# lmfaber/karma

Measured on AMD Instinct MI355X. Metric: contigs+reads/sec for k-mer vec + shared-read graph build; HBM GB/s vs roofline, higher is better.
Workload: dtype u32 keys / i64 counts / f64 div

## Files before the change

### include/karma.h

```cpp
#ifndef KARMA_H
#define KARMA_H

#include <stddef.h>
#include <stdint.h>

#ifdef __cplusplus
extern "C" {
#endif

#define KARMA_OK 0
#define KARMA_ERR_ARG (-1)
#define KARMA_ERR_KMER (-2)
#define KARMA_ERR_HIP (-3)
#define KARMA_ERR_OOM (-4)
#define KARMA_ERR_ZERO_DIV (-5)
#define KARMA_ERR_UNSORTED (-6)
#define KARMA_ERR_STATE (-7)
#define KARMA_ERR_PARSE (-8)
#define KARMA_ERR_COMM (-9)
#define KARMA_ERR_STALL (-10)

#define KARMA_KMER_5P6 (-1)

int karma_version(void);
// ... 79 lines not shown
int karma_ctx_join(karma_ctx* ctx, void* side);
int karma_ctx_set_side_headroom(karma_ctx* ctx, int blocks_per_cu);
int karma_kmer_row_totals(karma_kmer_plan* p, int64_t* dst_host);

typedef struct karma_pairs karma_pairs;
#define KARMA_REC_SORTED 0
#define KARMA_REC_UNSORTED 1
#define KARMA_REC_FLAGGED 2
int karma_graph_records(karma_ctx* ctx, const uint32_t* records, int64_t n_records, int64_t n_contigs, int flags,
                        int is_device, karma_pairs** out);
typedef struct karma_graph_job karma_graph_job;
int karma_graph_records_begin(karma_ctx* ctx, const uint32_t* records, int64_t n_records, int64_t n_contigs,
                              int flags, int is_device, karma_graph_job** job);
int karma_graph_records_end(karma_graph_job* job, karma_pairs** out);
int karma_graph_split_hint(karma_ctx* ctx, const int64_t* bounds, int nranks);
int karma_graph_eq(karma_ctx* ctx, const int64_t* cls_off, const uint32_t* members, const int64_t* counts,
                   const uint8_t* pair_skip, int64_t n_classes, int64_t n_contigs, int is_device, karma_pairs** out);
int karma_graph_eq_compact(karma_ctx* ctx, const uint8_t* sizes, const uint32_t* members, int64_t n_members,
                           const uint32_t* counts, int64_t C, int64_t n_contigs, karma_pairs** out);
int karma_pairs_merge(karma_ctx* ctx, const uint64_t* keys, const int64_t* counts, int64_t n, int is_device,
                      karma_pairs** out);
int karma_pairs_merge_runs(karma_ctx* ctx, const uint64_t* keys, const int64_t* counts, const int64_t* run_off,
                           int n_runs, int is_device, karma_pairs** out);
int karma_pairs_get_kc(karma_pairs* p, int64_t* kc_dev);
int karma_pairs_merge_runs_kc(karma_ctx* ctx, const int64_t* kc_dev, const int64_t* run_off, int n_runs,
                              karma_pairs** out);
int karma_pairs_destroy(karma_pairs* p);
int karma_pairs_rebind(karma_pairs* p, karma_ctx* ctx);
int karma_pairs_count(karma_pairs* p, int64_t* n);
int karma_pairs_device(karma_pairs* p, const uint64_t** keys, const int64_t** counts);
// ... 105 lines not shown
```

### karma_amd/_lib.py

```python

from __future__ import annotations

import ctypes
import os
import weakref

import numpy as np

HERE = os.path.dirname(os.path.abspath(__file__))
LIB_PATH = os.environ.get("KARMA_LIB") or os.path.join(HERE, "libkarma_hip.so")

KARMA_OK = 0
KARMA_ERR_ARG = -1
KARMA_ERR_KMER = -2
KARMA_ERR_HIP = -3
KARMA_ERR_OOM = -4
KARMA_ERR_ZERO_DIV = -5
KARMA_ERR_UNSORTED = -6
KARMA_ERR_STATE = -7
KARMA_ERR_PARSE = -8
KARMA_ERR_COMM = -9
KARMA_ERR_STALL = -10

KARMA_DT_U8, KARMA_DT_I32, KARMA_DT_I64, KARMA_DT_U64, KARMA_DT_F64 = 0, 1, 2, 3, 4
# ... 67 lines not shown
    "karma_kmer_exceptions_set": [_c_p, _c_p, _i64],
    "karma_kmer_plan_finalize": [_c_p, _I64P],
    "karma_kmer_plan_finalize_async": [_c_p],
    "karma_kmer_plan_finalize_wait": [_c_p, _I64P],
    "karma_kmer_columns": [_c_p, _c_p],
    "karma_kmer_profile": [_c_p, _c_p, _i64, _i32],
    "karma_kmer_profile_rows": [_c_p, _i64, _i64, _c_p, _i64, _i32],
    "karma_kmer_profile_side": [_c_p, _c_p, _i64, _c_p],
    "karma_ctx_join": [_c_p, _c_p],
    "karma_ctx_set_side_headroom": [_c_p, _i32],
    "karma_kmer_row_totals": [_c_p, _c_p],
    "karma_graph_records": [_c_p, _c_p, _i64, _i64, _i32, _i32, _PP],
    "karma_graph_records_begin": [_c_p, _c_p, _i64, _i64, _i32, _i32, _PP],
    "karma_graph_records_end": [_c_p, _PP],
    "karma_graph_split_hint": [_c_p, _c_p, _i32],
    "karma_graph_eq": [_c_p, _c_p, _c_p, _c_p, _c_p, _i64, _i64, _i32, _PP],
    "karma_graph_eq_compact": [_c_p, _c_p, _c_p, _i64, _c_p, _i64, _i64, _PP],
    "karma_pairs_merge": [_c_p, _c_p, _c_p, _i64, _i32, _PP],
    "karma_pairs_merge_runs": [_c_p, _c_p, _c_p, _c_p, _i32, _i32, _PP],
    "karma_pairs_merge_runs_kc": [_c_p, _c_p, _c_p, _i32, _PP],
    "karma_pairs_get_kc": [_c_p, _c_p],
    "karma_pairs_destroy": [_c_p],
    "karma_pairs_rebind": [_c_p, _c_p],
    "karma_pairs_count": [_c_p, _I64P],
    "karma_pairs_device": [_c_p, _PP, _PP],
    "karma_pairs_get": [_c_p, _c_p, _c_p, _c_p, _i32],
    "karma_pairs_split": [_c_p, _c_p, _i32, _c_p],
    "karma_pairs_totals": [_c_p, _c_p, _i64],
    "karma_edges_from_pairs": [_c_p, _c_p, _i32, _c_p, _i64, _PP, _I64P],
    "karma_edges_begin": [_c_p, _c_p, _i32, _i64, _PP, _PP],
# ... 309 lines not shown
```

### karma_amd/csrc/graph_sets.hip

```cpp

#include <algorithm>
#include <cstdlib>
#include <cstring>
#include <memory>
#include <type_traits>

#include "karma_internal.h"
#include "sets_ctrl.h"

using namespace karma;

namespace {

#include "graph_device.h"

typedef unsigned int u32x4 __attribute__((ext_vector_type(4)));

constexpr int kMaxB = 2048;
constexpr int kMaxBc = 512;
constexpr int kNarrowB = 512, kNarrowBc = 128;
constexpr int kCrSmax = 64;
constexpr int kCrPieces = 512;
constexpr int kCgShift = 18;
constexpr int kOneGroupB = 128;
// ... 134 lines not shown
                                               uint32_t* m0_out) {
    const uint32_t za = (uint32_t)__builtin_ctz(a.win), zb = (uint32_t)__builtin_ctz(b.win);
    const uint32_t ma = a.fm3 + za, mb = b.fm3 + zb, m0 = min(ma, mb);
    const uint32_t rel = ((a.win >> za) << min(ma - m0, 31u)) | ((b.win >> zb) << min(mb - m0, 31u));
    *code = K23 ? m0 << 4 | rel : m0 | (rel >> 1) << 24;
    *m0_out = m0;
    return COMPACT ? lanes(rel < 16u) & (K23 ? ~0ull : lanes(m0 < N)) : 0ull;
}

__device__ __forceinline__ uint32_t dpp_shr1(uint32_t old, uint32_t v) {
    return (uint32_t)__builtin_amdgcn_update_dpp((int)old, (int)v, 0x138, 0xF, 0xF, false);
}

constexpr int kRareMax = int(kCChunk / kCIter);
constexpr int kRareW = 5;
#ifndef KARMA_CLS_PACKED
#define KARMA_CLS_PACKED 0
#endif
constexpr int kCls2Waves = 4;

constexpr int kBinQ = 64;
constexpr int kBinMaxBc = 56;
constexpr int kBinHdr = 4;
struct BinArgs {
    uint16_t* segs;
    uint4* hdr;
    uint8_t* dir;
    int64_t seg_cap;
    int dir_cap;
    int slotted;
};

template <bool HIST, bool COMPACT, bool REMAP = false, bool BIN = false, bool FLAG = false>
__global__ void __launch_bounds__(kCW) __attribute__((amdgpu_waves_per_eu(kCls2Waves, kCls2Waves)))
classify2_kernel(ClassArgs P, BinArgs Q) {
    static_assert(!(HIST && BIN), "the binned classify has no partition block histograms");
    auto PA = [&]() -> const ClassArgs& {
        const char* ka = (const char*)__builtin_amdgcn_kernarg_segment_ptr();
        asm volatile("" : "+s"(ka));
        return *reinterpret_cast<const ClassArgs*>(ka);
    };
    constexpr int RPL = FLAG ? 16 : 8;
    constexpr int64_t kIt = 64 * RPL;
    constexpr int kFPer = RPL / 4;
    static_assert(!FLAG || kFPer <= kCPer, "the step's units fit the register set");
    constexpr bool RC = BIN && FLAG;
    constexpr bool RAW = FLAG;
    constexpr bool PK = RC && KARMA_CLS_PACKED;
    constexpr uint32_t kWinTop = PK ? 7u : 31u;
    const int lane = threadIdx.x & 63;
    const int wave = __builtin_amdgcn_readfirstlane(threadIdx.x >> 6);
    const int64_t chunk = P.c0 + (int64_t)blockIdx.x * (kCW / 64) + wave;
    const int64_t c_lo = chunk * P.chunk;
    if (c_lo >= P.A) return;
    const int64_t c_hi = min(P.A, c_lo + P.chunk);
    uint32_t* out = P.codes + c_lo;
    const uint64_t out_u = (uint64_t)out;
    const __amdgpu_buffer_rsrc_t out_rsrc = __builtin_amdgcn_make_buffer_rsrc(
        reinterpret_cast<void*>(((uint64_t)(uint32_t)__builtin_amdgcn_readfirstlane((int)(out_u >> 32)) << 32) |
                                (uint32_t)__builtin_amdgcn_readfirstlane((int)(uint32_t)out_u)),
        0, (int)(P.chunk * 4), 0x00020000);
    constexpr int kRows = BIN ? 32 : 64;
    __shared__ __attribute__((aligned(16))) u32x4 tbuf[kCW / 64][kRows * 4];
    u32x4* tb = tbuf[wave];
    __shared__ uint32_t whist[kCW / 64][HIST ? kMaxBc : 1];
    uint32_t* wh = whist[wave];
    __shared__ __attribute__((aligned(16))) uint16_t bq[kCW / 64][BIN ? kBinMaxBc * kBinQ : 8];
    __shared__ uint32_t bcnt[kCW / 64][BIN ? kBinMaxBc : 1];
    uint16_t* const q = bq[wave];
    uint32_t* const qn = bcnt[wave];
    __shared__ uint32_t bback[kCW / 64][BIN ? 8 : 1];
    uint32_t* const bst = bback[wave];
    __shared__ uint32_t rlist[kCW / 64][kRareMax * kRareW];
    uint32_t* const rl = rlist[wave];
    uint32_t n_rare = 0;
    constexpr bool hist_on = HIST;
    if (hist_on) {
        for (int b = lane; b < P.Bc; b += 64) wh[b] = 0;
        wave_sync();
    }
    if (BIN) {
        if (lane < P.Bc) qn[lane] = 0;
        if (lane < 8) bst[lane] = 0;
        wave_sync();
// ... 27 lines not shown
            }
            if (lane == 0) {
                Qa.dir[chunk * Qa.dir_cap + nbk] = (uint8_t)fb;
                bst[0] = nbk + 1;
                bst[1 + (fb >> 5)] |= 1u << (fb & 31);
                if (nbk < 16) bst[3 + (nbk >> 2)] |= fb << (8 * (nbk & 3));
            }
            wave_lds_order();
            if (in_mask(over) && bk == fb) q[fb * kBinQ + pos - kBinQ] = val;
            if (lane == 0) qn[fb] -= (uint32_t)kBinQ;
            wave_lds_order();
        }
    };
    uint32_t* const stg = reinterpret_cast<uint32_t*>(tb);
    const uint32_t* const stg_l = stg + lane;
    uint32_t ns = 0;
    uint32_t nc = 0, ng = 0;
    auto stage = [&](uint64_t b, uint32_t v) {
        if (in_mask(b)) stg[ns + (uint32_t)rank_below(b)] = v;
        ns += __popcll(b);
    };
    static_assert(kBinQ == 64, "queue slots: bk << 6");
    uint64_t stage_hi = 0, hi_next = 0;
    const uint32_t code_hi = ((uint32_t)max(P.N, 3u) - 3u) << 4;
    auto bin_stage = [&]() {
        if (!ns) return;
        wave_lds_order();
        for (uint32_t j0 = 0; j0 < ns; j0 += 64) {
            uint32_t cd = stg_l[j0];
            uint64_t m = lanes((uint32_t)lane < ns - j0);
// ... 60 lines not shown
#pragma unroll
            for (int u = 0; u < kFPer; ++u) b[u] = u32x4{rm(b[u].x), rm(b[u].y), rm(b[u].z), rm(b[u].w)};
            return;
        }
#pragma unroll
        for (int u = 0; u < kCPer; ++u) {
            b[u].y = b[u].y < P.N ? P.remap[b[u].y] : b[u].y;
            b[u].w = b[u].w < P.N ? P.remap[b[u].w] : b[u].w;
        }
    };
    auto step = [&](auto full_tag, auto replay_tag, u32x4 (&buf)[kCPer], u32x4 (&nxt)[kCPer], int64_t t0) {
        constexpr bool FULL = decltype(full_tag)::value;
        constexpr bool REPLAY = decltype(replay_tag)::value;
        uint32_t rid[RPL], ctg[RPL];
        if constexpr (FLAG) {
            const int rl = lane & 31;
#pragma unroll
            for (int h = 0; h < 2; ++h) {
#pragma unroll
                for (int u = 0; u < 2; ++u) {
                    const int g = 64 * u + lane;
                    tb[g ^ ((g >> 4) & 3)] = buf[2 * h + u];
                }
                wave_sync();
                if ((lane >> 5) == h) {
#pragma unroll
                    for (int k = 0; k < 4; ++k) {
                        const int g = 4 * rl + k;
                        const u32x4 qv = tb[g ^ ((g >> 4) & 3)];
                        rid[4 * k] = qv.x, rid[4 * k + 1] = qv.y, rid[4 * k + 2] = qv.z, rid[4 * k + 3] = qv.w;
                    }
                }
                wave_sync();
            }
#pragma unroll
            for (int i = 0; i < RPL; ++i) ctg[i] = rid[i] & kContigMask;
        } else if (!BIN) {
#pragma unroll
            for (int u = 0; u < kCPer; ++u) {
                const int row = 16 * u + (lane >> 2);
// ... 103 lines not shown
            auto S = [&](int i) -> uint64_t {
                if (FLAG) return lanes((int)rid[i] < 0) | (i == 0 && !have_prev ? 1ull : 0ull);
                return i == 0 ? lanes(rid[0] != prev_last) | (have_prev ? 0ull : 1ull) : lanes(rid[i] != rid[i - 1]);
            };
            const uint64_t S0 = S(0);
            RState hd;
            rs_reset(st, ctg[0]);
            hd = st;
            spos = 0;
            uint32_t hlen = in_mask(S0) ? 0u : (uint32_t)RPL;
            constexpr bool HLEN = RARE || RPL <= 8;
            started = S0;
            uint64_t Si = S0;
#pragma unroll
            for (int i = 0; i < RPL; ++i) {
                if (!RARE && BIN && i == 8) bin_stage();
                if (i > 0) {
                    const uint64_t cap = Si & ~started;
                    hd.win = in_mask(cap) ? st.win : hd.win;
                    if (HLEN) hlen = in_mask(cap) ? (uint32_t)i : hlen;
                    started |= Si;
                    spos = in_mask(Si) ? (uint32_t)i : spos;
                    if (RAW) {
                        const uint32_t w = rid[i];
                        const uint32_t fm3 = in_mask(Si) ? w - 0x80000003u : st.fm3;
                        st.win = in_mask(Si) ? 8u : st.win | (1u << min(w - fm3, kWinTop));
                        st.fm3 = fm3;
                    } else {
                        const uint32_t c = ctg[i];
                        const uint32_t fm3 = in_mask(Si) ? c - 3u : st.fm3;
                        st.win = (in_mask(Si) ? 0u : st.win) | (1u << min(c - fm3, 31u));
// ... 208 lines not shown
        }
        if (lane == 0) {
            uint4* const h = Q.hdr + kBinHdr * chunk;
            h[0] = uint4{0u, 0u, 0u, 0u};
            h[1] = uint4{0u, 0u, 0u, bst[0]};
            h[2] = uint4{bst[1], bst[2], bst[3], bst[4]};
            h[3] = uint4{bst[5], bst[6], nc, 0u};
        }
    } else if (BIN) {
        wave_lds_order();
        const uint32_t cnt = lane < P.Bc ? qn[lane] : 0u;
        const uint32_t g = (cnt + 7u) >> 3;
        const uint32_t incl = wave_scan_incl(g), excl = incl - g;
        const uint32_t G = lane63(incl);
        uint16_t* const gt = reinterpret_cast<uint16_t*>(tb);
        uint8_t* const gb = reinterpret_cast<uint8_t*>(tb) + 1024;
        for (uint32_t i = 0; i < g; ++i) gt[excl + i] = (uint16_t)(lane << 3 | i);
        gb[lane] = (uint8_t)g;
        wave_lds_order();
        for (uint32_t k0 = 0; k0 < G; k0 += 64) {
            const uint32_t k = k0 + lane;
            if (k < G) {
                const uint32_t e = gt[k], bk = e >> 3, i = e & 7u;
                const uint32_t n = qn[bk];
                u32x4 v = *reinterpret_cast<const u32x4*>(q + bk * kBinQ + 8 * i);
                const int k0c = 8 * (int)i;
                auto pad = [&](uint32_t w, int c) -> uint32_t {
                    const uint32_t lo = k0c + c < (int)n ? (w & 0xFFFFu) : 0xFFFFu;
                    const uint32_t hi = k0c + c + 1 < (int)n ? (w >> 16) : 0xFFFFu;
                    return lo | hi << 16;
                };
// ... 1439 lines not shown
int64_t chunk_records(const karma_ctx* ctx, int64_t A) {
    if (const char* e = std::getenv("KARMA_CHUNK")) {
        const int64_t c = std::atoll(e);
        if (c == kCChunk || c == kCChunk / 2 || c == kCChunk / 4) return c;
    }
    const int64_t slots = (int64_t)ctx->cu_count * 16;
    return ceil_div(A, kCChunk) < 4 * slots ? kCChunk / 2 : kCChunk;
}
int mark_at(int asked) {
    static const int env = [] {
        const char* e = std::getenv("KARMA_MARK_AT");
        return e ? std::atoi(e) : -1;
    }();
    return env >= 0 ? env : asked >= 0 ? asked : kMarkAt;
}
template <typename F>
int pick(bool b, F f) {
    return b ? f(std::true_type{}) : f(std::false_type{});
}
struct SetsJob {
    karma_ctx* ctx = nullptr;
    RecIn rec;
    int64_t A = 0, N = 0;
    SetsOpts opts;
    Geo g{};
    int B = 0;
    int64_t n_chunks = 0;
    int64_t chunk = kCChunk;
    bool wide_c = false, wide_p = false, append = false;
    int lpb = 0;
    int64_t n_pblk = 0;
    DevArray<uint32_t> codes, n_codes, n_gen, n_pl;
    DevArray<int64_t> big_list;
// ... 83 lines not shown
    lb = reinterpret_cast<uint64_t*>(cb + cl.lb);
    flags = reinterpret_cast<int*>(cb + cl.flags);
    counters = reinterpret_cast<unsigned*>(cb + cl.counters);
    n_per = cb + cl.n_per;
    dst = cb + cl.dst;
    ovf = reinterpret_cast<uint8_t*>(cb + cl.ovf);
    split_loc = cb + cl.split_loc;
    if (!deferred) {
        void* hpin = nullptr;
        KARMA_TRY(ctx_job_pinned(ctx, cl.readback * 8, &hpin));
        hctrl = static_cast<const int64_t*>(hpin);
    }
    max_cflush = n_pblk + ceil_div(A, CodeStream::kCap) + 1;
    ccap = A + max_cflush * (8 * (int64_t)g.Bc + 8);
    if (append) KARMA_TRY(blk_hist.alloc(ctx, n_pblk * g.Bc));
    bin = !append && g.Bc > 0 && g.Bc <= kBinMaxBc && bin_on();
    if (bin) {
        dir_cap = (int)(chunk / kBinQ);
        seg_cap = (uint32_t)(dir_cap + g.Bc);
        constexpr int kBinSlotMin = 120;
        slotted = A > 0 && chunk >= (int64_t)kBinSlotMin * g.Bc;
        KARMA_CHECK(n_chunks * (int64_t)seg_cap < (int64_t(1) << 32), KARMA_ERR_ARG,
                    "binned classify: %lld chunks exceed 32-bit segment indices", (long long)n_chunks);
        KARMA_TRY(bsegs.alloc(ctx, n_chunks * (int64_t)seg_cap * kBinQ));
        KARMA_TRY(bhdr.alloc(ctx, n_chunks * 4 * kBinHdr));
        KARMA_TRY(bdir.alloc(ctx, n_chunks * (int64_t)dir_cap));
    } else if (g.Bc > 0) {
        KARMA_TRY(cent.alloc(ctx, ccap + 16));
        KARMA_TRY(cf_base.alloc(ctx, max_cflush));
        KARMA_TRY(cf_off.alloc(ctx, max_cflush * (g.Bc + 1)));
    }
// ... 20 lines not shown
    const int64_t pscap = n_chunks * pcap + max_pflush * (4 * (int64_t)B + 4);
    KARMA_TRY(plist.alloc(ctx, n_chunks * pcap));
    KARMA_TRY(pent.alloc(ctx, pscap + 8));
    KARMA_TRY(pf_base.alloc(ctx, max_pflush));
    KARMA_TRY(pf_off.alloc(ctx, max_pflush * (B + 1)));
    const bool fresh_ext = ext && attempt == 0 && !relabeled;
    const bool probe = A > 0 && !relabeled && !fresh_ext;
    if (!probe && !fresh_ext) KARMA_HIP(hipMemsetAsync(cb, 0, cl.total * 8, ctx->stream));
    if (append) KARMA_HIP(hipMemsetAsync(blk_hist.ptr, 0, n_pblk * g.Bc * 4, ctx->stream));
    const int mark_here = mark_at(opts.mark);
    auto mark = [&](int at) -> int {
        if (mark_here != at || attempt != 0) return KARMA_OK;
        if (!ctx->mark_ev) KARMA_HIP(hipEventCreateWithFlags(&ctx->mark_ev, hipEventDisableTiming));
        KARMA_HIP(hipEventRecord(ctx->mark_ev, ctx->stream));
        ctx->mark_set = true;
        return KARMA_OK;
    };
    if (!relabeled) KARMA_TRY(mark(3));
    if (A > 0) {
        ClassArgs C{rec.pr,    A,         (uint32_t)N,   g.Bc > 0,     codes.ptr, n_codes.ptr,
                    n_gen.ptr, blk_items, lpb, big_list.ptr, counters, flags,
                    append ? blk_hist.ptr : nullptr, g.bwc, g.Bc, relabeled ? remap_map.ptr : nullptr, 0, nullptr,
                    chunk};
        C.recw = rec.fw;
        const BinArgs Bn = bin ? BinArgs{bsegs.ptr, reinterpret_cast<uint4*>(bhdr.ptr), bdir.ptr, (int64_t)seg_cap,
                                         dir_cap, slotted ? 1 : 0}
                               : BinArgs{};
        auto classify = [&](int64_t c_from, int64_t c_to) -> int {
            C.c0 = c_from;
            const int64_t cg = ceil_div(c_to - c_from, kCW / 64);
            if (cg <= 0) return KARMA_OK;
            return pick(rec.flagged(), [&](auto fl) -> int {
                auto go = [&](auto ap, auto bn) -> int {
                    return pick(relabeled, [&](auto rl) -> int {
                        KARMA_LAUNCH(ctx, "graph_classify",
                                     (classify2_kernel<decltype(ap)::value, true, decltype(rl)::value,
                                                       decltype(bn)::value, decltype(fl)::value>),
                                     cg, kCW, 0, C, Bn);
                        return KARMA_OK;
                    });
                };
                return bin ? go(std::false_type{}, std::true_type{})
                           : append ? go(std::true_type{}, std::false_type{}) : go(std::false_type{}, std::false_type{});
            });
        };
        if (probe) {
            KARMA_LAUNCH(ctx, "relabel_probe", relabel_probe_kernel, 1, kRelabelProbes, 0, rec, A, (uint32_t)N,
                         counters + kCtrRelabel, reinterpret_cast<uint64_t*>(cb), cl.total);
            C.skip = counters + kCtrRelabel;
        } else if (fresh_ext) {
            C.skip = counters + kCtrRelabel;
            C.vote = counters + kCtrVote;
        }
        KARMA_TRY(classify(0, n_chunks));
    }
    KARMA_TRY(mark(1));
    if (A == 0) {
        KARMA_HIP(hipMemsetAsync(n_codes.ptr, 0, n_chunks * 4, ctx->stream));
// ... 288 lines not shown
void sets_release(SetsJob* job) {
    if (!job) return;
    job->ctx->job_open = false;
    job->ctx->mark_set = false;
    delete job;
}

int records_to_pairs_sets(karma_ctx* ctx, RecIn rec, int64_t A, int64_t N, karma_pairs* out) {
    if (N > kMaxCompactN) return records_to_pairs_wide(ctx, rec, A, N, out);
    SetsJob* job = nullptr;
    KARMA_TRY(sets_begin(ctx, rec, A, N, SetsOpts{}, &job));
    return sets_end(job, out);
}

}
```

### karma_amd/csrc/karma_internal.h

```cpp
#pragma once

#include <hip/hip_runtime.h>

#include <cstdint>
#include <cstdio>
#include <map>
#include <string>
#include <utility>
#include <vector>

#include "../../include/karma.h"

namespace karma {

void set_error(const char* fmt, ...);

extern thread_local uint64_t t_hip_calls;
constexpr bool counted_call(const char* e) {
    return !((e[0] == 'h' && e[1] == 'i' && e[2] == 'p' && e[3] == 'G' && e[4] == 'e' && e[5] == 't' && e[6] == 'L') ||
             (e[0] == 'h' && e[1] == 'i' && e[2] == 'p' && e[3] == 'S' && e[4] == 'e' && e[5] == 't' && e[6] == 'D'));
}

#define KARMA_HIP(expr)                                                                     \
    do {                                                                                    \
// ... 181 lines not shown
namespace karma {
struct RecIn {
    const uint2* pr = nullptr;
    const uint32_t* fw = nullptr;
    __host__ __device__ bool flagged() const { return fw != nullptr; }
    __device__ __forceinline__ uint32_t contig(int64_t i) const { return fw ? fw[i] & 0x7FFFFFFFu : pr[i].y; }
    __device__ __forceinline__ bool cont(int64_t i) const { return fw ? (int)fw[i] >= 0 : pr[i].x == pr[i - 1].x; }
};
int records_to_pairs_sets(karma_ctx* ctx, RecIn rec, int64_t A, int64_t N, karma_pairs* out);
struct SetsOpts {
    hipStream_t fork = nullptr;
    bool single_stream = false;
    int mark = -1;
    int64_t* ctrl = nullptr;
    int64_t ctrl_words = 0;
};
struct SetsJob;
int64_t sets_max_contigs();
int sets_begin(karma_ctx* ctx, RecIn rec, int64_t A, int64_t N, const SetsOpts& opts, SetsJob** job);
int sets_end(SetsJob* job, karma_pairs* out);
void sets_free(SetsJob* job);
struct SetsDeferred {
    const uint64_t* keys = nullptr;
    const int64_t* counts = nullptr;
    int64_t cap = 0;
    const int64_t* dst = nullptr;
    const int64_t* split_loc = nullptr;
    std::vector<int64_t> split_b;
    int B = 0, bw = 0;
    const int* flags = nullptr;
// ... 12 lines not shown
```

### karma_amd/csrc/step.hip

```cpp
#include <algorithm>
#include <chrono>
#include <cstdlib>
#include <cstring>
#include <deque>
#include <initializer_list>
#include <memory>
#include <thread>
#include <vector>

#include "karma_internal.h"
#include "sets_ctrl.h"
#include "step_schedule.h"

using namespace karma;

namespace {

constexpr int kRing = 64;
constexpr int kLag = 3;

enum StepErr : int64_t { kErrOrder = 1, kErrRange = 2, kErrPartition = 4, kErrZeroTotal = 8, kErrMergeOrder = 16 };
struct StepStatus {
    uint64_t seq;
    int64_t slow;
// ... 496 lines not shown
    int64_t* graves_h = nullptr;
    hipEvent_t grave_ev[kRing] = {};
    std::deque<int> graves;
    int grave_next = 0;
    int64_t n_sync = 0, n_deferred = 0, n_redone = 0;
    int64_t run_ns = 0, wait_ns = 0;
    karma_contigs* acgt_store = nullptr;
    int64_t kc = 0;
    bool defer_ranks = true;
    bool xstream = true;
    hipEvent_t ev_rec = nullptr, ev_sync = nullptr, ev_tail[2] = {};
    bool tail_set[2] = {}, sync_set = false;
    int tail_last = -1;
    bool one_comm = true;
    hipEvent_t ev_pres = nullptr, ev_pres2 = nullptr, ev_pre = nullptr;
    int64_t n_two = 0, n_xs = 0, n_own = 0;
    int stall_s = 120;
    int lag = kLag;
    void* ring_mem = nullptr;
    uint64_t fault_seq = 0;
};

namespace {

int sync_all(std::initializer_list<hipStream_t> order, bool quiet = false) {
    for (hipStream_t q : order) {
        if (!q) continue;
        if (quiet) (void)hipStreamSynchronize(q);
        else KARMA_HIP(hipStreamSynchronize(q));
    }
// ... 117 lines not shown
    DevArray<int64_t> send, all;
    KARMA_TRY(send.alloc(ctx, mx));
    KARMA_TRY(all.alloc(ctx, mx * W));
    const int64_t mine = b[s->rank + 1] - b[s->rank];
    if (mine)
        KARMA_HIP(hipMemcpyAsync(send.ptr, buf + b[s->rank], mine * 8, hipMemcpyDeviceToDevice, ctx->stream));
    KARMA_TRY(karma_comm_allgather(s->comm, send.ptr, all.ptr, mx * 8));
    for (int r = 0; r < W; ++r) {
        const int64_t n = b[r + 1] - b[r];
        if (r != s->rank && n)
            KARMA_HIP(hipMemcpyAsync(buf + b[r], all.ptr + r * mx, n * 8, hipMemcpyDeviceToDevice, ctx->stream));
    }
    return KARMA_OK;
}

int stream_after(hipEvent_t* ev, hipStream_t on, hipStream_t w) {
    if (!*ev) KARMA_HIP(hipEventCreateWithFlags(ev, hipEventDisableTiming));
    KARMA_HIP(hipEventRecord(*ev, on));
    return wait_event(w, *ev);
}

int run_sync(karma_step* s, karma_contigs* store, const uint32_t* rec, int64_t A, bool flg, bool keep,
             bool sequential, bool count) {
    const int rfmt = flg ? KARMA_REC_FLAGGED : KARMA_REC_SORTED;
    karma_ctx* ctx = s->ctx;
    KARMA_TRY(drop_outputs(s));
    ++s->n_sync;
    if (s->tail_last >= 0) {
        KARMA_TRY(wait_event(s->main_s, s->ev_tail[s->tail_last]));
    }
    if (s->world > 1 && s->one_comm && !sequential) {
        KARMA_TRY(stream_after(&s->ev_pre, s->main_s, s->side_s));
    }
// ... 150 lines not shown
                s->prof_par = newest_par;
                s->prof_M = newest_M;
                s->M = s->E = -1;
            }
        }
    }
    return KARMA_OK;
}

struct StepStreams {
    hipStream_t records, side, tail, xs, fork;
};

using JobGuard = std::unique_ptr<SetsJob, void (*)(SetsJob*)>;

int deferred_records(karma_step* s, const DeferredSchedule& sc, const StepStreams& q, karma_step::Tail& tl,
                     const uint32_t* rec, int64_t A, bool flg, JobGuard& jg, SetsDeferred* v) {
    karma_ctx* ctx = s->ctx;
    StreamScope on_records(ctx, q.records);
    if (s->exchange) KARMA_TRY(karma_graph_split_hint(ctx, s->bounds.data(), s->nranks));
    SetsOpts jo;
    jo.single_stream = sc.single_stream;
    jo.fork = q.fork;
    jo.mark = sc.mark;
    jo.ctrl = tl.ctrl.ptr;
    jo.ctrl_words = (int64_t)tl.ctrl.n;
    RecIn rin;
    if (flg) rin.fw = rec;
    else rin.pr = reinterpret_cast<const uint2*>(rec);
    SetsJob* job = nullptr;
    KARMA_TRY(sets_begin_deferred(ctx, rin, A, s->n_glob, jo, &job, v));
    jg.reset(job);
    if (v->ctrl) {
        ++s->n_own;
        return KARMA_OK;
    }
    KARMA_TRY(sync_all({s->side_s, s->side_alt_s, s->main_s, s->alt_s}));
    KARMA_TRY(tl.ctrl.alloc(ctx, (size_t)(v->ctrl_need + v->ctrl_need / 4 + 64)));
    KARMA_HIP(hipMemsetAsync(tl.ctrl.ptr, 0, tl.ctrl.n * 8, q.records));
    return KARMA_OK;
}

int deferred_profile(karma_step* s, const DeferredSchedule& sc, const StepStreams& q, karma_step::Tail& tl,
                     karma_contigs* store, uint64_t seq, bool sequential) {
    karma_ctx* ctx = s->ctx;
    StreamScope on_side(ctx, q.side);
    DevArray<uint32_t>& pz = s->plan_zero[sc.plan_zero];
    PlanOpts po;
    if (!sequential) {
        if (!pz.ptr) {
            KARMA_TRY(pz.alloc(ctx, 2048 + 2));
            KARMA_HIP(hipMemsetAsync(pz.ptr, 0, pz.n * 4, q.side));
        }
        po.zeroed = pz.ptr;
        po.zeroed_words = (int64_t)pz.n;
    }
    karma_kmer_plan* plan = nullptr;
    int rc = kmer_plan_create(ctx, store, s->kmode, po, &plan);
    if (!rc && s->world > 1) {
// ... 4 lines not shown
                s->sync_set = false;
            }
            {
                StreamScope on_xs(ctx, q.xs);
                if (!rc) rc = exchange_presence(s, plan, s->comm);
                if (!rc) rc = stream_after(&s->ev_pres2, q.xs, q.side);
            }
        } else {
            rc = exchange_presence(s, plan, s->scomm ? s->scomm : s->comm);
        }
    }
    int64_t* const m_dev = s->m_ring.ptr + seq % kRing;
    if (!rc) rc = kmer_finalize_device(plan, m_dev, s->mring_d + seq % kRing);
    if (rc && !sequential && pz.ptr) (void)hipMemsetAsync(pz.ptr, 0, pz.n * 4, q.side);
    if (!rc) rc = ensure_prof(s, tl.prof, (size_t)std::max<int64_t>(1, s->n_loc * kmer_m_cap(plan)));
    if (!rc && ctx->mark_set && !sequential) rc = wait_event(q.side, ctx->mark_ev);
    if (!rc && s->n_loc) rc = kmer_profile_device_m(plan, tl.prof.ptr, m_dev);
    if (plan) karma_kmer_plan_destroy(plan);
    return rc;
}

int deferred_tail(karma_step* s, const DeferredSchedule& sc, const StepStreams& q, karma_step::Tail& tl,
                  const SetsDeferred& v, uint64_t seq) {
    karma_ctx* ctx = s->ctx;
    if (sc.xs_on) {
        KARMA_TRY(stream_after(&s->ev_rec, q.records, q.xs));
        if (s->sync_set) {
            KARMA_TRY(stream_after(&s->ev_sync, s->main_s, q.xs));
            s->sync_set = false;
        }
    }
    StreamScope on_tail(ctx, q.tail);
    const uint64_t* lk = v.keys;
    const int64_t* lc = v.counts;
// ... 97 lines not shown
    const DeferredSchedule sc =
        deferred_schedule({s->world, s->xstream, s->one_comm, s->streams, A, sequential, flg, seq});
    hipStream_t const by_role[] = {nullptr, s->main_s, s->alt_s, s->side_s, s->side_alt_s};
    auto on = [&](StreamRole r) { return by_role[(int)r]; };
    const StepStreams q{on(sc.records), on(sc.side), on(sc.tail), on(kExchangeStream), on(sc.fork)};
    if (sc.two) ++s->n_two;
    if (sc.xs_on) ++s->n_xs;
    if (s->tail_set[sc.par]) KARMA_TRY(wait_event(q.records, s->ev_tail[sc.par]));
    karma_step::Tail& tl = s->tail[sc.par];
    FailGuard fail{s, tl, seq};
    s->prof_seq = seq;
    s->prof_par = sc.par;
    s->prof_M = -1;
    JobGuard job(nullptr, sets_release);
    SetsDeferred v;
    KARMA_TRY(deferred_records(s, sc, q, tl, rec, A, flg, job, &v));
    KARMA_TRY(deferred_profile(s, sc, q, tl, store, seq, sequential));
    KARMA_TRY(deferred_tail(s, sc, q, tl, v, seq));
    fail.armed = false;
    s->pending.push_back({seq, store, rec, A, flg});
    return KARMA_OK;
}

}

extern "C" {

int karma_step_create(karma_ctx* ctx, karma_comm* comm, karma_comm* side_comm, int kmode, int64_t n_glob,
                      const int64_t* bounds, int nranks, int rank, karma_step** out) {
    KARMA_TRY(ctx_begin(ctx));
    KARMA_CHECK(out && bounds && nranks >= 1 && nranks <= kMaxRuns && rank >= 0 && rank < nranks && n_glob >= 1,
                KARMA_ERR_ARG, "karma_step_create: bad arguments (nranks %d, rank %d)", nranks, rank);
// ... 192 lines not shown
    if (totals) KARMA_HIP(hipMemcpyAsync(totals, tl.tot.ptr, s->n_glob * 8, kind, q));
    KARMA_HIP(hipStreamSynchronize(q));
    return KARMA_OK;
}

int karma_step_destroy(karma_step* s) {
    if (!s) return KARMA_OK;
    hipSetDevice(s->ctx->device);
    (void)sync_all({s->main_s, s->alt_s, s->side_s, s->side_alt_s}, true);
    s->pending.clear();
    s->E = 0;
    drop_outputs(s);
    bury(s, true);
    for (auto& ev : s->grave_ev)
        if (ev) hipEventDestroy(ev);
    for (hipEvent_t ev : {s->ev_rec, s->ev_sync, s->ev_tail[0], s->ev_tail[1], s->ev_pres, s->ev_pres2, s->ev_pre})
        if (ev) hipEventDestroy(ev);
    if (s->graves_h) hipHostFree(s->graves_h);
    if (s->ring_mem) hipHostFree(s->ring_mem);
    s->prof.release();
    s->m_ring.release();
    s->plan_zero[0].release();
    s->plan_zero[1].release();
    for (auto& tl : s->tail) tl.release();
    karma_ctx* ctx = s->ctx;
    hipStream_t prev = ctx->stream;
    if (prev == s->main_s || prev == s->side_s || prev == s->alt_s || prev == s->side_alt_s)
        ctx->stream = ctx->own_stream;
    if (s->side_alt_s) karma_stream_destroy(ctx, s->side_alt_s);
    if (s->side_s) karma_stream_destroy(ctx, s->side_s);
    if (s->alt_s) karma_stream_destroy(ctx, s->alt_s);
// ... 7 lines not shown
```

### karma_amd/csrc/step_schedule.h

```cpp
#pragma once
#include <cstdint>

namespace karma {

constexpr int kMarkOne = 2;
constexpr int kMarkTwo = 4;
constexpr int kMarkOneFlagged = 2;
constexpr int64_t kAltMaxRecords = int64_t(1) << 27;

enum class StreamRole : int { kNone = 0, kMain = 1, kAlt = 2, kSide = 3, kSideAlt = 4 };

constexpr StreamRole kExchangeStream = StreamRole::kSideAlt;

struct ScheduleIn {
    int world = 1;
    bool xstream = true;
    bool one_comm = true;
    int streams = 0;
    int64_t A = 0;
    bool sequential = false;
    bool flg = false;
    uint64_t seq = 0;
};

struct DeferredSchedule {
    bool two = false;
    bool xs_on = false;
    int par = 0;
    StreamRole records = StreamRole::kMain;
    StreamRole side = StreamRole::kSide;
    StreamRole tail = StreamRole::kMain;
    StreamRole fork = StreamRole::kNone;
    bool single_stream = false;
    int mark = kMarkOne;
    int plan_zero = 0;
};

inline DeferredSchedule deferred_schedule(const ScheduleIn& in) {
    DeferredSchedule d;
    d.two = (in.world == 1 || (in.xstream && !in.sequential)) &&
            (in.streams ? in.streams == 2 : in.A < kAltMaxRecords);
    d.xs_on = !in.sequential && in.xstream && in.world > 1 && (d.two || in.one_comm);
    d.par = in.sequential || !d.two ? 0 : (int)(in.seq & 1);
    d.records = d.par ? StreamRole::kAlt : StreamRole::kMain;
    d.side = in.sequential ? d.records : d.par && !d.xs_on ? StreamRole::kSideAlt : StreamRole::kSide;
    d.tail = d.xs_on ? kExchangeStream : d.records;
    d.single_stream = d.two;
    d.fork = d.two ? StreamRole::kNone : StreamRole::kAlt;
    d.mark = d.two ? kMarkTwo : in.flg ? kMarkOneFlagged : kMarkOne;
    d.plan_zero = d.side == StreamRole::kSideAlt ? 1 : 0;
    return d;
}

}
```

Baseline: 129.0 billion.

## Pack binned flagged classify, size its LDS dynamically, and hook profile launch at mark

Makes packed windows the default for the binned flagged classify kernel. That kernel now takes a per-launch dynamic LDS queue sized by Bc and a smaller transpose buffer, split into four transpose passes, and its waves-per-EU bound is raised to allow more occupancy. A callback at the classify mark now issues the k-mer profile work from inside the records job, so the side stream is queued earlier and the records stream waits on a passed event. It also adds an occupancy query API. The risks are register pressure from the packed path and extra cross-stream dependencies.

Result: faster. 131.4 billion, median of 6 (+1.9%).

```diff
diff --git a/include/karma.h b/include/karma.h
--- a/include/karma.h
+++ b/include/karma.h
@@ -117,6 +117,7 @@
                               int flags, int is_device, karma_graph_job** job);
 int karma_graph_records_end(karma_graph_job* job, karma_pairs** out);
 int karma_graph_split_hint(karma_ctx* ctx, const int64_t* bounds, int nranks);
+int karma_graph_classify_occupancy(karma_ctx* ctx, int64_t n_contigs, int rec_format, int* blocks_per_cu);
 int karma_graph_eq(karma_ctx* ctx, const int64_t* cls_off, const uint32_t* members, const int64_t* counts,
                    const uint8_t* pair_skip, int64_t n_classes, int64_t n_contigs, int is_device, karma_pairs** out);
 int karma_graph_eq_compact(karma_ctx* ctx, const uint8_t* sizes, const uint32_t* members, int64_t n_members,
diff --git a/karma_amd/_lib.py b/karma_amd/_lib.py
--- a/karma_amd/_lib.py
+++ b/karma_amd/_lib.py
@@ -105,6 +105,7 @@
     "karma_graph_records_begin": [_c_p, _c_p, _i64, _i64, _i32, _i32, _PP],
     "karma_graph_records_end": [_c_p, _PP],
     "karma_graph_split_hint": [_c_p, _c_p, _i32],
+    "karma_graph_classify_occupancy": [_c_p, _i64, _i32, ctypes.POINTER(ctypes.c_int)],
     "karma_graph_eq": [_c_p, _c_p, _c_p, _c_p, _c_p, _i64, _i64, _i32, _PP],
     "karma_graph_eq_compact": [_c_p, _c_p, _c_p, _i64, _c_p, _i64, _i64, _PP],
     "karma_pairs_merge": [_c_p, _c_p, _c_p, _i64, _i32, _PP],
diff --git a/karma_amd/csrc/graph_sets.hip b/karma_amd/csrc/graph_sets.hip
--- a/karma_amd/csrc/graph_sets.hip
+++ b/karma_amd/csrc/graph_sets.hip
@@ -172,10 +172,8 @@
 
 constexpr int kRareMax = int(kCChunk / kCIter);
 constexpr int kRareW = 5;
-#ifndef KARMA_CLS_PACKED
-#define KARMA_CLS_PACKED 0
-#endif
 constexpr int kCls2Waves = 4;
+constexpr int kCls2BinWaves = 5;
 
 constexpr int kBinQ = 64;
 constexpr int kBinMaxBc = 56;
@@ -190,7 +188,8 @@
 };
 
 template <bool HIST, bool COMPACT, bool REMAP = false, bool BIN = false, bool FLAG = false>
-__global__ void __launch_bounds__(kCW) __attribute__((amdgpu_waves_per_eu(kCls2Waves, kCls2Waves)))
+__global__ void __launch_bounds__(kCW)
+    __attribute__((amdgpu_waves_per_eu(kCls2Waves, BIN && FLAG ? kCls2BinWaves : kCls2Waves)))
 classify2_kernel(ClassArgs P, BinArgs Q) {
     static_assert(!(HIST && BIN), "the binned classify has no partition block histograms");
     auto PA = [&]() -> const ClassArgs& {
@@ -204,7 +203,7 @@
     static_assert(!FLAG || kFPer <= kCPer, "the step's units fit the register set");
     constexpr bool RC = BIN && FLAG;
     constexpr bool RAW = FLAG;
-    constexpr bool PK = RC && KARMA_CLS_PACKED;
+    constexpr bool PK = RC;
     constexpr uint32_t kWinTop = PK ? 7u : 31u;
     const int lane = threadIdx.x & 63;
     const int wave = __builtin_amdgcn_readfirstlane(threadIdx.x >> 6);
@@ -218,14 +217,14 @@
         reinterpret_cast<void*>(((uint64_t)(uint32_t)__builtin_amdgcn_readfirstlane((int)(out_u >> 32)) << 32) |
                                 (uint32_t)__builtin_amdgcn_readfirstlane((int)(uint32_t)out_u)),
         0, (int)(P.chunk * 4), 0x00020000);
-    constexpr int kRows = BIN ? 32 : 64;
+    constexpr int kRows = BIN ? (FLAG ? 16 : 32) : 64;
     __shared__ __attribute__((aligned(16))) u32x4 tbuf[kCW / 64][kRows * 4];
     u32x4* tb = tbuf[wave];
     __shared__ uint32_t whist[kCW / 64][HIST ? kMaxBc : 1];
     uint32_t* wh = whist[wave];
-    __shared__ __attribute__((aligned(16))) uint16_t bq[kCW / 64][BIN ? kBinMaxBc * kBinQ : 8];
+    extern __shared__ __attribute__((aligned(16))) uint16_t cls_bq[];
     __shared__ uint32_t bcnt[kCW / 64][BIN ? kBinMaxBc : 1];
-    uint16_t* const q = bq[wave];
+    uint16_t* const q = cls_bq + (BIN ? wave * P.Bc * kBinQ : 0);
     uint32_t* const qn = bcnt[wave];
     __shared__ uint32_t bback[kCW / 64][BIN ? 8 : 1];
     uint32_t* const bst = bback[wave];
@@ -283,6 +282,9 @@
     };
     uint32_t* const stg = reinterpret_cast<uint32_t*>(tb);
     const uint32_t* const stg_l = stg + lane;
+    constexpr int kStgCap = kRows * 16;
+    constexpr int kStgPts = kStgCap / 64;
+    static_assert(!BIN || (kStgPts >= 1 && RPL % kStgPts == 0), "the staged codes of kStgPts emit points fit");
     uint32_t ns = 0;
     uint32_t nc = 0, ng = 0;
     auto stage = [&](uint64_t b, uint32_t v) {
@@ -373,16 +375,18 @@
         constexpr bool REPLAY = decltype(replay_tag)::value;
         uint32_t rid[RPL], ctg[RPL];
         if constexpr (FLAG) {
-            const int rl = lane & 31;
-#pragma unroll
-            for (int h = 0; h < 2; ++h) {
-#pragma unroll
-                for (int u = 0; u < 2; ++u) {
+            constexpr int kPass = BIN ? 4 : 2, kUP = kFPer / kPass, kPL = 64 / kPass;
+            static_assert(kFPer == 4 && kUP * 64 <= kRows * 4, "a pass fits the transpose buffer");
+            const int rl = lane & (kPL - 1);
+#pragma unroll
+            for (int h = 0; h < kPass; ++h) {
+#pragma unroll
+                for (int u = 0; u < kUP; ++u) {
                     const int g = 64 * u + lane;
-                    tb[g ^ ((g >> 4) & 3)] = buf[2 * h + u];
+                    tb[g ^ ((g >> 4) & 3)] = buf[kUP * h + u];
                 }
                 wave_sync();
-                if ((lane >> 5) == h) {
+                if (lane / kPL == h) {
 #pragma unroll
                     for (int k = 0; k < 4; ++k) {
                         const int g = 4 * rl + k;
@@ -516,7 +520,7 @@
             uint64_t Si = S0;
 #pragma unroll
             for (int i = 0; i < RPL; ++i) {
-                if (!RARE && BIN && i == 8) bin_stage();
+                if (!RARE && BIN && i > 0 && i % kStgPts == 0) bin_stage();
                 if (i > 0) {
                     const uint64_t cap = Si & ~started;
                     hd.win = in_mask(cap) ? st.win : hd.win;
@@ -755,7 +759,8 @@
         const uint32_t incl = wave_scan_incl(g), excl = incl - g;
         const uint32_t G = lane63(incl);
         uint16_t* const gt = reinterpret_cast<uint16_t*>(tb);
-        uint8_t* const gb = reinterpret_cast<uint8_t*>(tb) + 1024;
+        static_assert(kBinMaxBc * 8 * 2 + 64 <= kRows * 64, "the flush's tables fit the transpose buffer");
+        uint8_t* const gb = reinterpret_cast<uint8_t*>(tb) + kBinMaxBc * 8 * 2;
         for (uint32_t i = 0; i < g; ++i) gt[excl + i] = (uint16_t)(lane << 3 | i);
         gb[lane] = (uint8_t)g;
         wave_lds_order();
@@ -2225,9 +2230,24 @@
     }();
     return env >= 0 ? env : asked >= 0 ? asked : kMarkAt;
 }
+size_t class_bin_lds(int Bc) { return (size_t)(kCW / 64) * (size_t)Bc * kBinQ * sizeof(uint16_t); }
 template <typename F>
 int pick(bool b, F f) {
     return b ? f(std::true_type{}) : f(std::false_type{});
+}
+bool class_binned(int Bc) { return Bc > 0 && Bc < kAppendMinBc && Bc <= kBinMaxBc && bin_on(); }
+template <typename F>
+int with_classify(bool flagged, bool append, bool bin, bool relabeled, F f) {
+    return pick(flagged, [&](auto fl) -> int {
+        auto go = [&](auto ap, auto bn) -> int {
+            return pick(relabeled, [&](auto rl) -> int {
+                return f(&classify2_kernel<decltype(ap)::value, true, decltype(rl)::value, decltype(bn)::value,
+                                           decltype(fl)::value>);
+            });
+        };
+        return bin ? go(std::false_type{}, std::true_type{})
+                   : append ? go(std::true_type{}, std::false_type{}) : go(std::false_type{}, std::false_type{});
+    });
 }
 struct SetsJob {
     karma_ctx* ctx = nullptr;
@@ -2341,7 +2361,7 @@
     max_cflush = n_pblk + ceil_div(A, CodeStream::kCap) + 1;
     ccap = A + max_cflush * (8 * (int64_t)g.Bc + 8);
     if (append) KARMA_TRY(blk_hist.alloc(ctx, n_pblk * g.Bc));
-    bin = !append && g.Bc > 0 && g.Bc <= kBinMaxBc && bin_on();
+    bin = class_binned(g.Bc);
     if (bin) {
         dir_cap = (int)(chunk / kBinQ);
         seg_cap = (uint32_t)(dir_cap + g.Bc);
@@ -2392,6 +2412,11 @@
         if (!ctx->mark_ev) KARMA_HIP(hipEventCreateWithFlags(&ctx->mark_ev, hipEventDisableTiming));
         KARMA_HIP(hipEventRecord(ctx->mark_ev, ctx->stream));
         ctx->mark_set = true;
+        if (opts.at_mark) {
+            hipEvent_t passed = nullptr;
+            KARMA_TRY(opts.at_mark(opts.at_mark_arg, &passed));
+            if (passed) KARMA_HIP(hipStreamWaitEvent(ctx->stream, passed, 0));
+        }
         return KARMA_OK;
     };
     if (!relabeled) KARMA_TRY(mark(3));
@@ -2408,18 +2433,9 @@
             C.c0 = c_from;
             const int64_t cg = ceil_div(c_to - c_from, kCW / 64);
             if (cg <= 0) return KARMA_OK;
-            return pick(rec.flagged(), [&](auto fl) -> int {
-                auto go = [&](auto ap, auto bn) -> int {
-                    return pick(relabeled, [&](auto rl) -> int {
-                        KARMA_LAUNCH(ctx, "graph_classify",
-                                     (classify2_kernel<decltype(ap)::value, true, decltype(rl)::value,
-                                                       decltype(bn)::value, decltype(fl)::value>),
-                                     cg, kCW, 0, C, Bn);
-                        return KARMA_OK;
-                    });
-                };
-                return bin ? go(std::false_type{}, std::true_type{})
-                           : append ? go(std::true_type{}, std::false_type{}) : go(std::false_type{}, std::false_type{});
+            return with_classify(rec.flagged(), append, bin, relabeled, [&](auto kern) -> int {
+                KARMA_LAUNCH(ctx, "graph_classify", kern, cg, kCW, bin ? class_bin_lds(g.Bc) : 0, C, Bn);
+                return KARMA_OK;
             });
         };
         if (probe) {
@@ -2738,3 +2754,20 @@
 }
 
 }
+
+extern "C" int karma_graph_classify_occupancy(karma_ctx* ctx, int64_t n_contigs, int rec_format,
+                                              int* blocks_per_cu) {
+    using namespace karma;
+    KARMA_CHECK(ctx && blocks_per_cu && n_contigs >= 1 && n_contigs <= kMaxCompactN, KARMA_ERR_ARG,
+                "karma_graph_classify_occupancy: bad arguments (n_contigs %lld)", (long long)n_contigs);
+    KARMA_TRY(ctx_begin(ctx));
+    Geo g{};
+    KARMA_TRY(make_geo(n_contigs, &g));
+    const bool bin = class_binned(g.Bc);
+    const size_t lds = bin ? class_bin_lds(g.Bc) : 0;
+    return with_classify(rec_format == KARMA_REC_FLAGGED, g.Bc >= kAppendMinBc, bin, false, [&](auto kern) -> int {
+        KARMA_HIP(hipOccupancyMaxActiveBlocksPerMultiprocessor(blocks_per_cu, reinterpret_cast<const void*>(kern),
+                                                               kCW, lds));
+        return KARMA_OK;
+    });
+}
diff --git a/karma_amd/csrc/karma_internal.h b/karma_amd/csrc/karma_internal.h
--- a/karma_amd/csrc/karma_internal.h
+++ b/karma_amd/csrc/karma_internal.h
@@ -219,6 +219,8 @@
     int mark = -1;
     int64_t* ctrl = nullptr;
     int64_t ctrl_words = 0;
+    int (*at_mark)(void* arg, hipEvent_t* passed) = nullptr;
+    void* at_mark_arg = nullptr;
 };
 struct SetsJob;
 int64_t sets_max_contigs();
diff --git a/karma_amd/csrc/step.hip b/karma_amd/csrc/step.hip
--- a/karma_amd/csrc/step.hip
+++ b/karma_amd/csrc/step.hip
@@ -534,6 +534,7 @@
     int tail_last = -1;
     bool one_comm = true;
     hipEvent_t ev_pres = nullptr, ev_pres2 = nullptr, ev_pre = nullptr;
+    hipEvent_t ev_passed = nullptr;
     int64_t n_two = 0, n_xs = 0, n_own = 0;
     int stall_s = 120;
     int lag = kLag;
@@ -681,9 +682,13 @@
     return KARMA_OK;
 }
 
-int stream_after(hipEvent_t* ev, hipStream_t on, hipStream_t w) {
+int record_event(hipEvent_t* ev, hipStream_t on) {
     if (!*ev) KARMA_HIP(hipEventCreateWithFlags(ev, hipEventDisableTiming));
     KARMA_HIP(hipEventRecord(*ev, on));
+    return KARMA_OK;
+}
+int stream_after(hipEvent_t* ev, hipStream_t on, hipStream_t w) {
+    KARMA_TRY(record_event(ev, on));
     return wait_event(w, *ev);
 }
 
@@ -864,8 +869,19 @@
 
 using JobGuard = std::unique_ptr<SetsJob, void (*)(SetsJob*)>;
 
+struct ProfileAtMark {
+    karma_step* s;
+    const DeferredSchedule* sc;
+    const StepStreams* q;
+    karma_step::Tail* tl;
+    karma_contigs* store;
+    uint64_t seq;
+    bool done = false;
+};
+int profile_at_mark(void* arg, hipEvent_t* passed);
+
 int deferred_records(karma_step* s, const DeferredSchedule& sc, const StepStreams& q, karma_step::Tail& tl,
-                     const uint32_t* rec, int64_t A, bool flg, JobGuard& jg, SetsDeferred* v) {
+                     const uint32_t* rec, int64_t A, bool flg, JobGuard& jg, SetsDeferred* v, ProfileAtMark* hook) {
     karma_ctx* ctx = s->ctx;
     StreamScope on_records(ctx, q.records);
     if (s->exchange) KARMA_TRY(karma_graph_split_hint(ctx, s->bounds.data(), s->nranks));
@@ -875,6 +891,10 @@
     jo.mark = sc.mark;
     jo.ctrl = tl.ctrl.ptr;
     jo.ctrl_words = (int64_t)tl.ctrl.n;
+    if (hook) {
+        jo.at_mark = profile_at_mark;
+        jo.at_mark_arg = hook;
+    }
     RecIn rin;
     if (flg) rin.fw = rec;
     else rin.pr = reinterpret_cast<const uint2*>(rec);
@@ -892,7 +912,7 @@
 }
 
 int deferred_profile(karma_step* s, const DeferredSchedule& sc, const StepStreams& q, karma_step::Tail& tl,
-                     karma_contigs* store, uint64_t seq, bool sequential) {
+                     karma_contigs* store, uint64_t seq, bool sequential, hipEvent_t* passed = nullptr) {
     karma_ctx* ctx = s->ctx;
     StreamScope on_side(ctx, q.side);
     DevArray<uint32_t>& pz = s->plan_zero[sc.plan_zero];
@@ -927,10 +947,20 @@
     if (!rc) rc = kmer_finalize_device(plan, m_dev, s->mring_d + seq % kRing);
     if (rc && !sequential && pz.ptr) (void)hipMemsetAsync(pz.ptr, 0, pz.n * 4, q.side);
     if (!rc) rc = ensure_prof(s, tl.prof, (size_t)std::max<int64_t>(1, s->n_loc * kmer_m_cap(plan)));
-    if (!rc && ctx->mark_set && !sequential) rc = wait_event(q.side, ctx->mark_ev);
+    if (!rc && ctx->mark_set && !sequential) {
+        rc = wait_event(q.side, ctx->mark_ev);
+        if (!rc && passed) rc = record_event(&s->ev_passed, q.side);
+        if (!rc && passed) *passed = s->ev_passed;
+    }
     if (!rc && s->n_loc) rc = kmer_profile_device_m(plan, tl.prof.ptr, m_dev);
     if (plan) karma_kmer_plan_destroy(plan);
     return rc;
+}
+
+int profile_at_mark(void* arg, hipEvent_t* passed) {
+    ProfileAtMark* const h = static_cast<ProfileAtMark*>(arg);
+    h->done = true;
+    return deferred_profile(h->s, *h->sc, *h->q, *h->tl, h->store, h->seq, false, passed);
 }
 
 int deferred_tail(karma_step* s, const DeferredSchedule& sc, const StepStreams& q, karma_step::Tail& tl,
@@ -1058,8 +1088,9 @@
     s->prof_M = -1;
     JobGuard job(nullptr, sets_release);
     SetsDeferred v;
-    KARMA_TRY(deferred_records(s, sc, q, tl, rec, A, flg, job, &v));
-    KARMA_TRY(deferred_profile(s, sc, q, tl, store, seq, sequential));
+    ProfileAtMark hook{s, &sc, &q, &tl, store, seq};
+    KARMA_TRY(deferred_records(s, sc, q, tl, rec, A, flg, job, &v, sc.profile_at_mark ? &hook : nullptr));
+    if (!hook.done) KARMA_TRY(deferred_profile(s, sc, q, tl, store, seq, sequential));
     KARMA_TRY(deferred_tail(s, sc, q, tl, v, seq));
     fail.armed = false;
     s->pending.push_back({seq, store, rec, A, flg});
@@ -1282,7 +1313,8 @@
     bury(s, true);
     for (auto& ev : s->grave_ev)
         if (ev) hipEventDestroy(ev);
-    for (hipEvent_t ev : {s->ev_rec, s->ev_sync, s->ev_tail[0], s->ev_tail[1], s->ev_pres, s->ev_pres2, s->ev_pre})
+    for (hipEvent_t ev : {s->ev_rec, s->ev_sync, s->ev_tail[0], s->ev_tail[1], s->ev_pres, s->ev_pres2, s->ev_pre,
+                          s->ev_passed})
         if (ev) hipEventDestroy(ev);
     if (s->graves_h) hipHostFree(s->graves_h);
     if (s->ring_mem) hipHostFree(s->ring_mem);
diff --git a/karma_amd/csrc/step_schedule.h b/karma_amd/csrc/step_schedule.h
--- a/karma_amd/csrc/step_schedule.h
+++ b/karma_amd/csrc/step_schedule.h
@@ -34,6 +34,7 @@
     bool single_stream = false;
     int mark = kMarkOne;
     int plan_zero = 0;
+    bool profile_at_mark = false;
 };
 
 inline DeferredSchedule deferred_schedule(const ScheduleIn& in) {
@@ -49,6 +50,7 @@
     d.fork = d.two ? StreamRole::kNone : StreamRole::kAlt;
     d.mark = d.two ? kMarkTwo : in.flg ? kMarkOneFlagged : kMarkOne;
     d.plan_zero = d.side == StreamRole::kSideAlt ? 1 : 0;
+    d.profile_at_mark = in.world == 1 && !in.sequential && !d.two;
     return d;
 }
 
```
